# SamsungLabs/fcaf3d

Measured on AMD Instinct MI355X. Metric: scenes/sec fwd+bwd, ScanNet 100k-pt 2cm voxels, 1/2/4/8 MI355X, higher is better.
Workload: dtype f32

## Files before the change

fcaf3d_amd/csrc/conv.hip:

```cpp
#include "fc_common.h"
#include "../../include/fcaf3d_hip.h"
#ifdef FC_TRACE
__device__ unsigned long long* g_trace_buf_lds;
__device__ int g_trace_cap_lds;
extern "C" int fc_debug_trace_lds(unsigned long long* buf, int cap) {
  FC_HIP(hipMemcpyToSymbol(HIP_SYMBOL(g_trace_buf_lds), &buf, sizeof(buf)));
  FC_HIP(hipMemcpyToSymbol(HIP_SYMBOL(g_trace_cap_lds), &cap, sizeof(cap)));
  return FC_OK;
}
#define TR_BUF g_trace_buf_lds
#define TR_CAP g_trace_cap_lds
#endif
#include "fc_trace.h"

typedef float f32x16 __attribute__((ext_vector_type(16)));
typedef float f32x2 __attribute__((ext_vector_type(2)));
typedef float f32x4 __attribute__((ext_vector_type(4)));

__device__ __attribute__((aligned(16))) float g_zero_row[64];

__device__ int g_fc_prio;
extern "C" int fc_debug_set_prio(int mode) {
  FC_HIP(hipMemcpyToSymbol(HIP_SYMBOL(g_fc_prio), &mode, sizeof(mode)));
  return FC_OK;
}

static int g_bf16_fast = 0;
extern "C" int fc_set_bf16_fast(int on) {
  g_bf16_fast = on ? 1 : 0;
  return FC_OK;
}

static int g_split_mode = 2;
static inline int split_mode() { return g_bf16_fast ? 0 : g_split_mode; }
extern "C" int fc_set_split_mode(int mode) {
  if (mode != 0 && mode != 2) return FC_EINVAL;
  g_split_mode = mode;
  return FC_OK;
}
extern "C" int fc_get_split_mode(void) { return split_mode(); }
static int g_h3r = 1;
extern "C" int fc_debug_set_h3r(int mode) {
  if (mode < 0 || mode > 2) return FC_EINVAL;
  g_h3r = mode;
  return FC_OK;
}

#include <mutex>
#include "conv_tile.h"
#include "conv_f32.h"
#include "wgrad_f32.h"
#include "conv_stem.h"
#include "conv_x6.h"
#include "wgrad_x6.h"
#include "conv_h3r.h"
#include "conv_route.h"
static inline RouteEnv route_env() { return {split_mode(), g_bf16_fast, g_h3r}; }

__global__ __launch_bounds__(256) void k_amax(const f32x4* __restrict__ x, int64_t n4, const float* __restrict__ tail, int ntail,
                                              unsigned* __restrict__ slot) {
  __shared__ unsigned wm[4];
  __shared__ int last_s;
  unsigned m = 0u;
  const int64_t stride = (int64_t)gridDim.x * 256;
  for (int64_t i = (int64_t)blockIdx.x * 256 + threadIdx.x; i < n4; i += 4 * stride) {
    f32x4 v[4];
#pragma unroll
    for (int q = 0; q < 4; ++q) v[q] = i + q * stride < n4 ? x[i + q * stride] : f32x4{0.f, 0.f, 0.f, 0.f};
#pragma unroll
    for (int q = 0; q < 4; ++q)
#pragma unroll
      for (int j = 0; j < 4; ++j) { const unsigned u = __float_as_uint(v[q][j]) & 0x7fffffffu; m = (u > m && u < 0x7f800000u) ? u : m; }
  }
  if (blockIdx.x == 0 && (int)threadIdx.x < ntail) { const unsigned u = __float_as_uint(tail[threadIdx.x]) & 0x7fffffffu; m = (u > m && u < 0x7f800000u) ? u : m; }
#pragma unroll
  for (int off = 32; off > 0; off >>= 1) { const unsigned o = (unsigned)__shfl_xor((int)m, off, 64); m = o > m ? o : m; }
  if ((threadIdx.x & 63) == 0) wm[threadIdx.x >> 6] = m;
  __syncthreads();
  if (threadIdx.x == 0) {
    unsigned b = wm[0];
    for (int w = 1; w < 4; ++w) b = wm[w] > b ? wm[w] : b;
    if (b > __hip_atomic_load(&slot[1], __ATOMIC_RELAXED, __HIP_MEMORY_SCOPE_AGENT)) atomicMax(&slot[1], b);
    __threadfence();
    last_s = atomicAdd(&slot[2], 1u) == gridDim.x - 1;
    if (last_s) {
      __threadfence();
      slot[0] = atomicExch(&slot[1], 0u);
      slot[2] = 0u;
    }
  }
}

constexpr int AMAX_RING = 2048;
static unsigned* g_amax_ring[16] = {};
static unsigned g_amax_next[16] = {};
static std::mutex g_amax_ring_mu;
static int amax_ring_slot(unsigned** slot) {
  int dev = 0;
  FC_HIP(hipGetDevice(&dev));
  if (dev < 0 || dev >= 16) return FC_EINVAL;
  std::lock_guard<std::mutex> lock(g_amax_ring_mu);
  if (!g_amax_ring[dev]) {
    FC_HIP(hipMalloc((void**)&g_amax_ring[dev], (size_t)AMAX_RING * FC_AMAX_SLOT_BYTES));
    FC_HIP(hipMemset(g_amax_ring[dev], 0, (size_t)AMAX_RING * FC_AMAX_SLOT_BYTES));
  }
  const unsigned i = __atomic_fetch_add(&g_amax_next[dev], 1u, __ATOMIC_RELAXED) % AMAX_RING;
  *slot = g_amax_ring[dev] + (size_t)i * (FC_AMAX_SLOT_BYTES / 4);
  return FC_OK;
}
static int amax_launch(const float* x, int64_t n, unsigned* slot, hipStream_t stream) {
// ... 410 lines not shown
template <int G>
__global__ __launch_bounds__(256) void k_wgrad_reduce4(const float* __restrict__ part, float* __restrict__ gW, int64_t elems4, int S) {
  __shared__ f32x4 red[256];
  constexpr int COLS = 256 / G;
  const int col = threadIdx.x % COLS, g = threadIdx.x / COLS;
  const int64_t i = (int64_t)blockIdx.x * COLS + col;
  const int per = (S + G - 1) / G;
  const int s0 = g * per, s1 = (s0 + per < S) ? s0 + per : S;
  f32x4 a = {0.f, 0.f, 0.f, 0.f};
  if (i < elems4) {
    const f32x4* src = reinterpret_cast<const f32x4*>(part) + i;
    int sl = s0;
    for (; sl + 4 <= s1; sl += 4) {
      const f32x4 v0 = src[(int64_t)sl * elems4], v1 = src[(int64_t)(sl + 1) * elems4];
      const f32x4 v2 = src[(int64_t)(sl + 2) * elems4], v3 = src[(int64_t)(sl + 3) * elems4];
      a += v0; a += v1; a += v2; a += v3;
    }
    for (; sl < s1; ++sl) a += src[(int64_t)sl * elems4];
  }
  if (G == 1) {
    if (i < elems4) reinterpret_cast<f32x4*>(gW)[i] = a;
    return;
  }
  red[threadIdx.x] = a;
  __syncthreads();
  if (g == 0 && i < elems4) {
    for (int q = 1; q < G; ++q) a += red[q * COLS + col];
    reinterpret_cast<f32x4*>(gW)[i] = a;
  }
}

__global__ void k_transpose_w(const float* __restrict__ W, float* __restrict__ Wt, int K, int Cin, int Cout) {
  __shared__ float tile[32][33];
  int k = blockIdx.z;
  int ci0 = blockIdx.y * 32, co0 = blockIdx.x * 32;
  int tx = threadIdx.x & 31, ty = threadIdx.x >> 5;
  for (int j = ty; j < 32; j += 8) {
    int ci = ci0 + j, co = co0 + tx;
    tile[j][tx] = (ci < Cin && co < Cout) ? W[((int64_t)k * Cin + ci) * Cout + co] : 0.f;
  }
  __syncthreads();
  for (int j = ty; j < 32; j += 8) {
    int co = co0 + j, ci = ci0 + tx;
    if (ci < Cin && co < Cout) Wt[((int64_t)k * Cout + co) * Cin + ci] = tile[tx][j];
  }
}

struct WgradArgs {
  const float *in, *gout; const int *nbr, *row_index, *cnt; float* part;
  int64_t n_out; int K, Cin, Cout; const unsigned *amax_in, *amax_gout; hipStream_t stream;
};
#define FC_LAUNCH(...) __VA_ARGS__<<<grid, 256, 0, a.stream>>>(a.in, a.gout, a.nbr, a.row_index, a.cnt, a.part, a.n_out, a.K, a.Cin, a.Cout, r.rps)
#define FC_LAUNCH_X6T(...) __VA_ARGS__<<<grid, 256, 0, a.stream>>>(a.in, a.gout, a.nbr, a.row_index, a.cnt, a.part, a.n_out, a.K, a.Cin, a.Cout, r.rps, a.amax_in, a.amax_gout, r.wbuf)
#define FC_LAUNCH_TABLE(...) __VA_ARGS__<<<grid, 256, 0, a.stream>>>(a.in, a.gout, a.nbr, a.part, a.n_out, a.K, a.Cin, a.Cout, r.rps)

template <int BM, int BN, int KO, bool PAIRS>
static void launch_wgrad_x6t(const WgradRoute& r, const WgradArgs& a, dim3 grid) {
  if (r.mode == FC_MODE_BF16) FC_LAUNCH_X6T(k_wgrad_x6t<BM, BN, KO, PAIRS, 1>);
  else if (r.mode == FC_MODE_H3) FC_LAUNCH_X6T(k_wgrad_x6t<BM, BN, KO, PAIRS, 2>);
  else FC_LAUNCH_X6T(k_wgrad_x6t<BM, BN, KO, PAIRS>);
}

template <int BM, int BN>
static void launch_wgrad_tile(const WgradRoute& r, const WgradArgs& a, dim3 grid) {
  const bool pairs = r.table == FC_TABLE_PAIRS;
  if (r.family == FC_WFAM_X6T) { if (pairs) launch_wgrad_x6t<BM, BN, 1, true>(r, a, grid); else launch_wgrad_x6t<BM, BN, 1, false>(r, a, grid); }
  else if (r.family == FC_WFAM_MFMA && !pairs && r.bkr == 32) { if (a.nbr) FC_LAUNCH(k_wgrad_mfma<BM, BN, true, 32, false>); else FC_LAUNCH(k_wgrad_mfma<BM, BN, false, 32, false>); }
  else if constexpr (BM == 64) {
    if (r.family == FC_WFAM_MFMA) { if (pairs) FC_LAUNCH(k_wgrad_mfma<64, BN, true, 32, true>); else FC_LAUNCH(k_wgrad_mfma<64, BN, true, 64, false>); }
    else if (pairs) FC_LAUNCH(k_wgrad_mfma_p<BN, true, true>);
    else if (a.nbr) FC_LAUNCH(k_wgrad_mfma_p<BN, true, false>);
    else FC_LAUNCH(k_wgrad_mfma_p<BN, false, false>);
  }
}

static int launch_wgrad(const WgradRoute& r, const WgradArgs& a) {
  const dim3 grid((unsigned)r.S, r.grid_y);
  const bool wide = r.bn == 128;
  if (r.family == FC_WFAM_STEM) {
    const size_t smem = (size_t)(STEM_ROWS * STEM_JP + STEM_ROWS * 64) * sizeof(float);
    k_stem_wgrad<<<(unsigned)r.S, 256, smem, a.stream>>>(a.in, a.gout, a.nbr, a.part, a.n_out, a.K, r.rps);
  } else if (r.family == FC_WFAM_FMA) FC_LAUNCH_TABLE(k_wgrad_fma);
  else if (r.family == FC_WFAM_MULTI) { if (wide) FC_LAUNCH_TABLE(k_wgrad_multi<128, WGRAD_KO>); else FC_LAUNCH_TABLE(k_wgrad_multi<64, WGRAD_KO>); }
  else if (r.ko == WGRAD_KO) { if (wide) launch_wgrad_x6t<64, 128, WGRAD_KO, false>(r, a, grid); else launch_wgrad_x6t<64, 64, WGRAD_KO, false>(r, a, grid); }
  else if (r.bm == 128) { if (wide) launch_wgrad_tile<128, 128>(r, a, grid); else launch_wgrad_tile<128, 64>(r, a, grid); }
  else { if (wide) launch_wgrad_tile<64, 128>(r, a, grid); else launch_wgrad_tile<64, 64>(r, a, grid); }
  FC_CHECK_LAUNCH();
  return FC_OK;
}
#undef FC_LAUNCH
#undef FC_LAUNCH_X6T
#undef FC_LAUNCH_TABLE

extern "C" {

static int wgrad_reduce(const float* part, float* gW, int64_t elems, int S, hipStream_t stream) {
  if (elems % 4 == 0) {
    const int64_t e4 = elems / 4;
    if (S >= 64) k_wgrad_reduce4<16><<<(unsigned)fc_cdiv(e4, 16), 256, 0, stream>>>(part, gW, e4, S);
    else if (S >= 16) k_wgrad_reduce4<4><<<(unsigned)fc_cdiv(e4, 64), 256, 0, stream>>>(part, gW, e4, S);
    else k_wgrad_reduce4<1><<<(unsigned)fc_cdiv(e4, 256), 256, 0, stream>>>(part, gW, e4, S);
  } else {
    k_wgrad_reduce<<<(unsigned)fc_cdiv(elems, 256), 256, 0, stream>>>(part, gW, elems, S);
  }
  FC_CHECK_LAUNCH();
  return FC_OK;
}

int fc_stem_conv_fwd(const float* in, const float* W, const int* nbr, float* out, float* col, int64_t n_in, int64_t n_out,
                     int K, hipStream_t stream) {
  if (n_in < 0 || n_out < 0 || K < 1 || K > 27 || !nbr) return FC_EINVAL;
  if (n_out == 0) return FC_OK;
  size_t smem = (size_t)(STEM_ROWS * STEM_FWD_LDA + 96 * 64) * sizeof(float);
  k_stem_fwd<<<(unsigned)fc_cdiv(n_out, STEM_ROWS), 256, smem, stream>>>(in, W, nbr, out, col, n_out, K);
  FC_CHECK_LAUNCH();
  return FC_OK;
}

static void stem_col_plan(int64_t n_out, int* S, int64_t* rps) {
  int64_t r = fc_cdiv(fc_cdiv(n_out > 0 ? n_out : 1, 192), STEM_ROWS) * STEM_ROWS;
  *rps = r;
  *S = (int)fc_cdiv(n_out > 0 ? n_out : 1, r);
}

int64_t fc_stem_conv_wgrad_ws_bytes(int64_t n_out, int K) {
  int S; int64_t rps;
  stem_col_plan(n_out, &S, &rps);
  return (int64_t)S * K * STEM_CIN * STEM_COUT * (int64_t)sizeof(float);
}

int fc_stem_conv_wgrad(const float* col, const float* gout, float* gW, int64_t n_out, int K, void* ws, int64_t ws_bytes,
                       hipStream_t stream) {
  if (n_out < 0 || K < 1 || K > 27) return FC_EINVAL;
  const int64_t elems = (int64_t)K * STEM_CIN * STEM_COUT;
  if (n_out == 0) {
    FC_HIP(hipMemsetAsync(gW, 0, elems * sizeof(float), stream));
    return FC_OK;
  }
  int S; int64_t rps;
  stem_col_plan(n_out, &S, &rps);
  if (ws_bytes < (int64_t)S * elems * (int64_t)sizeof(float)) return FC_EWS;
  float* part = (S == 1) ? gW : (float*)ws;
  size_t smem = (size_t)(STEM_ROWS * STEM_JP + STEM_ROWS * 64) * sizeof(float);
  k_stem_wgrad_col<<<(unsigned)S, 256, smem, stream>>>(col, gout, part, n_out, K, rps);
  FC_CHECK_LAUNCH();
  if (S > 1) return wgrad_reduce(part, gW, elems, S, stream);
  return FC_OK;
}

int fc_conv_wgrad_route(int64_t n_in, int64_t n_out, int K, int Cin, int Cout, int flags, int table_kind, int* out) {
  if (!out || n_in < 0 || n_out < 0 || K < 1 || Cin < 1 || Cout < 1) return FC_EINVAL;
  const WgradRoute r = wgrad_route({n_in, n_out, K, Cin, Cout}, flags, table_kind, route_env());
  const int f[16] = {r.family, r.bm, r.bn, r.ko, r.bkr, r.table, r.mode, r.S, (int)(r.rps < 0x7fffffff ? r.rps : 0x7fffffff), r.wbuf, (int)r.grid_y};
  for (int i = 0; i < 16; ++i) out[i] = f[i];
  return r.family == FC_WFAM_INVALID ? FC_EINVAL : FC_OK;
}

int64_t fc_conv_wgrad_ws_bytes(int64_t n_out, int K, int Cin, int Cout, int flags) {
  int S = 0;
  for (int table : {FC_TABLE_NONE, FC_TABLE_DENSE, FC_TABLE_PAIRS}) {
    const WgradRoute r = wgrad_route({n_out, n_out, K, Cin, Cout}, flags, table, route_env());
    if (r.family != FC_WFAM_INVALID && r.S > S) S = r.S;
  }
  return (int64_t)S * K * Cin * Cout * (int64_t)sizeof(float);
}

static int conv_wgrad_impl(const float* in, const float* gout, const int* nbr, const int* row_index, const int* cnt,
                           float* gW, int64_t n_in, int64_t n_out, int K, int Cin, int Cout, int flags, void* ws,
                           int64_t ws_bytes, hipStream_t stream) {
  AmaxHintScope hint_scope;
  if (n_in < 0 || n_out < 0 || K < 1 || Cin < 1 || Cout < 1) return FC_EINVAL;
  const int64_t elems = (int64_t)K * Cin * Cout;
  if (n_out == 0) { FC_HIP(hipMemsetAsync(gW, 0, elems * sizeof(float), stream)); return FC_OK; }
  const WgradRoute r = wgrad_route({n_in, n_out, K, Cin, Cout}, flags, cnt ? FC_TABLE_PAIRS : nbr ? FC_TABLE_DENSE : FC_TABLE_NONE, route_env());
  if (r.family == FC_WFAM_INVALID) return FC_EINVAL;
  if (ws_bytes < (int64_t)r.S * elems * (int64_t)sizeof(float)) return FC_EWS;
  WgradArgs a = {in, gout, nbr, row_index, cnt, (r.S == 1) ? gW : (float*)ws, n_out, K, Cin, Cout, nullptr, nullptr, stream};
  int rc = FC_OK;
  if (r.mode == FC_MODE_H3) {
    rc = operand_amax(in, n_in * (int64_t)Cin, 0, stream, &a.amax_in);
    if (rc == FC_OK) rc = operand_amax(gout, n_out * (int64_t)Cout, 1, stream, &a.amax_gout);
  }
  if (rc == FC_OK) rc = launch_wgrad(r, a);
  if (rc == FC_OK && r.S > 1) rc = wgrad_reduce(a.part, gW, elems, r.S, stream);
  return rc;
}

int fc_conv_wgrad(const float* in, const float* gout, const int* nbr, const int* row_index, float* gW, int64_t n_in,
                  int64_t n_out, int K, int Cin, int Cout, int flags, void* ws, int64_t ws_bytes, hipStream_t stream) {
  if (row_index) return FC_EINVAL;
  return conv_wgrad_impl(in, gout, nbr, nullptr, nullptr, gW, n_in, n_out, K, Cin, Cout, flags, ws, ws_bytes, stream);
}

int fc_conv_wgrad_pairs(const float* in, const float* gout, const int* pair_in, const int* pair_out, const int* pair_cnt,
                        float* gW, int64_t n_in, int64_t n_out, int K, int Cin, int Cout, int flags, void* ws,
                        int64_t ws_bytes, hipStream_t stream) {
  if (!pair_in || !pair_out || !pair_cnt) return FC_EINVAL;
  return conv_wgrad_impl(in, gout, pair_in, pair_out, pair_cnt, gW, n_in, n_out, K, Cin, Cout, flags, ws, ws_bytes, stream);
}

int fc_transpose_weight(const float* W, float* Wt, int K, int Cin, int Cout, hipStream_t stream) {
  if (K < 1 || Cin < 1 || Cout < 1 || K > 65535) return FC_EINVAL;
  dim3 grid((unsigned)fc_cdiv(Cout, 32), (unsigned)fc_cdiv(Cin, 32), (unsigned)K);
  k_transpose_w<<<grid, 256, 0, stream>>>(W, Wt, K, Cin, Cout);
  FC_CHECK_LAUNCH();
  return FC_OK;
// ... 4 lines not shown
```

fcaf3d_amd/csrc/conv_route.h:

```cpp
#ifndef FC_CONV_ROUTE_H
#define FC_CONV_ROUTE_H
#include "fc_common.h"
#include "../../include/fcaf3d_hip.h"

struct RouteEnv { int split_mode, bf16_fast, h3r; };
struct ConvShape { int64_t n_in, n_out; int K, Cin, Cout; };

struct ConvRoute {
  int family;
  int bm, bn, wm;
  int S;
  int wsrc, mode, buf, epi;
  unsigned grid[3];
};
struct WgradRoute {
  int family;
  int bm, bn, ko, bkr;
  int table, mode, S;
  int64_t rps;
  int wbuf;
  unsigned grid_y;
};

static inline int flag_bm(int flags) { return (flags >> FC_CONV_BM_SHIFT) & FC_CONV_TILE_MASK; }
static inline int flag_bn(int flags) { return (flags >> FC_CONV_BN_SHIFT) & FC_CONV_TILE_MASK; }
static inline int flag_s(int flags) { return (flags >> FC_CONV_S_SHIFT) & FC_CONV_S_MASK; }
static inline bool below_2gb(uint64_t bytes) { return bytes < (1ull << 31) - 4096u; }

static inline bool stem_shape(int K, int Cin, int Cout, int flags) { return !(flags & FC_CONV_FMA) && Cin == 3 && Cout == 64 && K <= 27; }

static inline int offset_split(int64_t tiles, int K) {
  if (K <= 1 || tiles >= 384) return 1;
  return (int)(1024 / tiles < K ? 1024 / tiles : K);
}

static inline ConvRoute conv_route(const ConvShape& s, int flags, int table, int64_t live_tiles, const RouteEnv& env) {
  const bool stats = (table & FC_TABLE_STATS) != 0;
  table &= ~FC_TABLE_STATS;
  const bool pairs = table == FC_TABLE_PAIRS, gather = table != FC_TABLE_NONE, split = (flags & FC_CONV_SPLIT) != 0;
  const bool image = split && (flags & FC_CONV_IMAGE);
  const bool wt = (flags & FC_CONV_WT) && !image;
  const int64_t n = s.n_out > 0 ? s.n_out : 1;
  const int K = s.K, Cin = s.Cin, Cout = s.Cout;
  ConvRoute r = {};
  r.family = FC_FAM_INVALID;
  r.wsrc = image ? FC_WSRC_IMAGE : wt ? FC_WSRC_FP32_T : FC_WSRC_FP32;
  if (!gather && (K != 1 || s.n_in != s.n_out)) return r;
  if ((flags & FC_CONV_WT) && !gather) return r;
  const bool mfma = Cin % 32 == 0 && Cout % 64 == 0 && (pairs || (!(flags & FC_CONV_FMA) && K <= 32));
  if (pairs && !mfma) return r;
  if (stats && !(mfma && split)) return r;
  r.bn = (Cout % 128 == 0) ? 128 : 64;
  if (pairs) {
    if (flag_bn(flags) == 1) r.bn = 64;
    r.bm = 128;
    r.S = K;
  } else {
    r.bm = (n > 64 && fc_cdiv(n, 128) * (Cout / r.bn) >= 4) ? 128 : 64;
    if (Cout == 64 && fc_cdiv(n, 256) >= 1024 && !split) r.bm = 256;
    const int fbm = flag_bm(flags), fbn = flag_bn(flags);
    if (fbm) r.bm = fbm == 1 ? 64 : (fbm == 2 ? 128 : 256);
    if (fbn && (Cout % (fbn == 1 ? 64 : 128) == 0)) r.bn = fbn == 1 ? 64 : 128;
    if (r.bm == 256) r.bn = 64;
    if (split && mfma && r.bm == 64) r.bm = 128;
    r.S = mfma ? offset_split(fc_cdiv(n, r.bm) * (Cout / r.bn), K) : 1;
    if (flag_s(flags)) r.S = flag_s(flags) > K ? K : flag_s(flags);
  }
  r.wm = r.bm == 256 ? 4 : 2;
  if (stem_shape(K, Cin, Cout, flags) && !(flags & FC_CONV_WT) && table == FC_TABLE_DENSE) { r.family = FC_FAM_STEM; return r; }
  if (!mfma && table != FC_TABLE_SORTED && !(flags & FC_CONV_IMAGE)) r.family = FC_FAM_FMA;
  if (!mfma) return r;
  r.grid[0] = (unsigned)fc_cdiv(n, r.bm), r.grid[1] = (unsigned)(Cout / r.bn), r.grid[2] = (unsigned)r.S;
  if (pairs && live_tiles > 0) r.grid[0] = (unsigned)live_tiles, r.grid[2] = 1;
  if (split) {
// ... 15 lines not shown
  if (r.family == FC_FAM_GLDS && wt) r.family = FC_FAM_MFMA;
  if (r.bm == 64) r.family = FC_FAM_MFMA;
  return r;
}

#define WGRAD_KO 3

static inline WgradRoute wgrad_route(const ConvShape& s, int flags, int table, const RouteEnv& env) {
  const int64_t n = s.n_out > 0 ? s.n_out : 1;
  const int K = s.K, Cin = s.Cin, Cout = s.Cout, fbm = flag_bm(flags), fbn = flag_bn(flags);
  const bool dense = table == FC_TABLE_DENSE, pairs = table == FC_TABLE_PAIRS, split = (flags & FC_CONV_SPLIT) != 0;
  if (pairs) flags &= ~FC_CONV_WGRAD_DEEP;
  WgradRoute r = {};
  r.family = FC_WFAM_INVALID;
  r.table = table, r.ko = 1, r.bkr = 32, r.mode = FC_MODE_FP32;
  if (table == FC_TABLE_SORTED || (table == FC_TABLE_NONE && (K != 1 || s.n_in != s.n_out))) return r;
  const bool mfma = !(flags & FC_CONV_FMA) && Cin % 64 == 0 && Cout % 64 == 0;
  if (pairs && !mfma) return r;
  if (stem_shape(K, Cin, Cout, flags)) {
    r.family = dense ? FC_WFAM_STEM : FC_WFAM_FMA;
    r.rps = 1024, r.S = (int)fc_cdiv(n, 1024), r.grid_y = dense ? 1 : (unsigned)K;
    return r;
  }
  const bool multi = dense && mfma && !(flags & FC_CONV_WGRAD_MULTI_OFF) && K % WGRAD_KO == 0 && n >= 4096 &&
                     (!(flags & FC_CONV_WGRAD_MULTI_FIRST) || (Cin == 64 && n >= 32768));
  const bool x6t = mfma && split && (multi || !dense);
  const int wide = (Cout % 128 == 0) ? 128 : 64;
  r.bm = 64;
  r.bn = wide;
  if (fbm == 2 && Cin % 128 == 0) r.bm = 128;
  if (fbn == 1) r.bn = 64;
  if (fbn == 2 && Cout % 128 == 0) r.bn = 128;
  if (split && !dense && Cin % 128 == 0) r.bm = 128;
  int64_t sp = 1728 / (mfma ? (int64_t)K * (Cin / r.bm) * (Cout / r.bn) : (int64_t)K);
  if (multi) {
    constexpr int round_wide = 256, round_narrow = 512;
    sp = (wide == 128 ? round_wide : round_narrow) / ((int64_t)(K / WGRAD_KO) * (Cin / 64) * (Cout / wide));
  }
  const int64_t max_by_rows = fc_cdiv(n, mfma ? 512 : 2048);
  sp = sp > max_by_rows ? max_by_rows : sp;
  sp = sp > 256 ? 256 : sp < 1 ? 1 : sp;
  if (flag_s(flags)) sp = flag_s(flags);
  r.rps = fc_align(fc_cdiv(n, sp), 64);
  r.S = (int)fc_cdiv(n, r.rps);
  if (!mfma) { r.family = FC_WFAM_FMA, r.grid_y = (unsigned)K; return r; }
  if (x6t) {
    r.family = FC_WFAM_X6T;
    r.mode = env.bf16_fast ? FC_MODE_BF16 : env.split_mode == 2 ? FC_MODE_H3 : FC_MODE_SIX;
    r.bn = wide;
    if (multi) r.bm = 64, r.ko = WGRAD_KO;
    else if (r.bm == 128 && r.bn == 128 && (int64_t)r.S * K * (Cin / 128) * (Cout / 128) < 512) r.bm = 64;
    r.wbuf = !(flags & FC_CONV_FLAT) && below_2gb((uint64_t)s.n_in * (uint64_t)Cin * 4u) && below_2gb((uint64_t)s.n_out * (uint64_t)Cout * 4u) &&
             s.n_in < (1 << 24) && s.n_out < (1 << 24) && below_2gb((uint64_t)K * (uint64_t)s.n_out * 4u);
  } else if (multi) {
    r.family = FC_WFAM_MULTI, r.bm = 64, r.bn = wide, r.ko = WGRAD_KO;
  } else {
    if (pairs) r.bm = 64;
    const bool wpipe = r.bm == 64 && !(flags & FC_CONV_WGRAD_DEEP) && !(flags & FC_CONV_WGRAD_PIPE_OFF) &&
                       ((flags & FC_CONV_WGRAD_PIPE_ON) || (pairs && r.bn == 128));
    r.family = wpipe ? FC_WFAM_MFMA_P : FC_WFAM_MFMA;
    if (!wpipe && dense && (flags & FC_CONV_WGRAD_DEEP) && r.bm == 64) r.bkr = 64;
  }
  r.grid_y = (unsigned)((K / r.ko) * (Cin / r.bm) * (Cout / r.bn));
  return r;
}
#endif
```

fcaf3d_amd/csrc/wgrad_x6.h:

```cpp
#pragma once

#ifdef FC_KO_WG_NOSPLIT
#define WG_SPLIT2(x0, x1, p0, p1, p2) do { p0 = x6_hi2(__float_as_uint(x0), __float_as_uint(x1)); p1 = p0; p2 = p0; } while (0)
#else
#define WG_SPLIT2(x0, x1, p0, p1, p2) x6_split2(x0, x1, p0, p1, p2)
#endif


typedef short x6_s16x4 __attribute__((ext_vector_type(4)));
__device__ __forceinline__ u32x4 x6_tr_frag(const u32x2* base, int unit) {
  const auto p = (__attribute__((address_space(3))) x6_s16x4*)(base + unit);
  const x6_s16x4 lo = __builtin_amdgcn_ds_read_tr16_b64_v4i16(p);
  const x6_s16x4 hi = __builtin_amdgcn_ds_read_tr16_b64_v4i16(p + 32);
  const u32x2 a = __builtin_bit_cast(u32x2, lo), b = __builtin_bit_cast(u32x2, hi);
  u32x4 v = {a[0], a[1], b[0], b[1]};
  return v;
}

template <int BMc, int BNc, int KO, bool PAIRS, int MODE = 0>
__global__ __launch_bounds__(256, (KO * (BMc / 64) * (BNc / 64) >= 6) ? 2 : 3) void k_wgrad_x6t(
    const float* __restrict__ in, const float* __restrict__ gout, const int* __restrict__ nbr,
    const int* __restrict__ row_index, const int* __restrict__ cnt, float* __restrict__ part, int64_t n_out, int K, int Cin,
    int Cout, int64_t rows_per_split, const unsigned* __restrict__ amax_a, const unsigned* __restrict__ amax_g, int buf) {
  constexpr int TM = BMc / 64, TN = BNc / 64;
// ... 177 lines not shown
#pragma unroll
                  for (int j = 0; j < TN; ++j) acc[o][i][j] = H3_MFMA(fa[o][pa][i], fb[pb][j], acc[o][i][j]);
        }
      } else
#pragma unroll
      for (int b = 0; b < 2; ++b) {
        u32x4 fb[3][TN];
#pragma unroll
        for (int pl = 0; pl < 3; ++pl)
#pragma unroll
          for (int j = 0; j < TN; ++j) fb[pl][j] = x6_tr_frag(Gs, (pl * SG + wc * TN + j) * 256 + b * 128 + f_unit);
        u32x4 fa[KO][3][TM];
#pragma unroll
        for (int o = 0; o < KO; ++o)
#pragma unroll
          for (int pl = 0; pl < 3; ++pl)
#pragma unroll
            for (int i = 0; i < TM; ++i) fa[o][pl][i] = x6_tr_frag(As, ((o * 3 + pl) * SA + wr * TM + i) * 256 + b * 128 + f_unit);
#pragma unroll
        for (int pb = 2; pb >= 0; --pb)
#pragma unroll
          for (int pa = 2 - pb; pa >= 0; --pa)
#pragma unroll
            for (int o = 0; o < KO; ++o)
#pragma unroll
              for (int i = 0; i < TM; ++i)
#pragma unroll
                for (int j = 0; j < TN; ++j) {
#ifdef FC_KO_WG_NOMFMA
                  acc[o][i][j][0] += __uint_as_float((fa[o][pa][i][0] ^ fb[pb][j][0]) & 0x3fffffu);
#else
                  acc[o][i][j] = X6_MFMA(fa[o][pa][i], fb[pb][j], acc[o][i][j]);
#endif
                }
      }
    }
  }
#pragma unroll
  for (int o = 0; o < KO; ++o) {
    if (k0 + o >= K) break;
    float* dst = part + ((int64_t)blockIdx.x * K + k0 + o) * Cin * Cout;
#pragma unroll
    for (int i = 0; i < TM; ++i)
#pragma unroll
      for (int j = 0; j < TN; ++j)
#pragma unroll
        for (int e = 0; e < 16; ++e) {
          const int row = ci0 + wr * (BMc / 2) + i * 32 + (e & 3) + 8 * (e >> 2) + 4 * h;
          const int col = co0 + wc * (BNc / 2) + j * 32 + r;
          dst[(int64_t)row * Cout + col] = H3 ? acc[o][i][j][e] * h3_inv : acc[o][i][j][e];
        }
  }
}
```

include/fcaf3d_hip.h:

```cpp
#ifndef FCAF3D_HIP_H
#define FCAF3D_HIP_H
#include <stdint.h>

#ifndef __HIP_PLATFORM_AMD__
typedef struct ihipStream_t* hipStream_t;
#endif

#ifdef __cplusplus
extern "C" {
#endif

#define FC_ABI_VERSION 19
#ifndef FC_AMAX_SLOT_BYTES
#define FC_AMAX_SLOT_BYTES 2048
#endif
int fc_abi_version(void);


int fc_voxelize(const float* points, int64_t n, int pt_stride, int batch_idx, float voxel_size, float feat_div,
                int nfeat, int* coords, float* feats, hipStream_t stream);

int fc_augment_voxelize(const float* points, int64_t n_src, int pt_stride, const int* sample_idx, int64_t n_out,
                        const float* xform_host, int batch_idx, float voxel_size, float feat_div, int nfeat, int* coords,
                        float* feats, float* points_out, hipStream_t stream);
// ... 85 lines not shown
int fc_conv_fwd(const float* in, const float* W, const int* nbr, const int* out_index, float* out, int64_t n_in,
                int64_t n_out, int K, int Cin, int Cout, int flags, void* ws, int64_t ws_bytes, hipStream_t stream);

int64_t fc_conv_fwd_pairs_ws_bytes(int64_t n_out, int K, int Cout);
int fc_conv_fwd_pairs(const float* in, const float* W, const int* pair_in, const int* pair_cnt, const int* pair_pos,
                      float* out, int64_t n_in, int64_t n_out, int K, int Cin, int Cout, int flags, void* ws,
                      int64_t ws_bytes, hipStream_t stream);

int fc_conv_fwd_pairs_tiles(const float* in, const float* W, const int* pair_in, const int* pair_cnt, const int* pair_pos,
                            float* out, int64_t n_in, int64_t n_out, int K, int Cin, int Cout, int64_t live_tiles, int flags,
                            void* ws, int64_t ws_bytes, hipStream_t stream);

int64_t fc_conv_stats_blocks(int64_t n_out, int K, int Cin, int Cout, int flags, int pairs);
int fc_conv_fwd_stats(const float* in, const float* W, const int* nbr, const int* out_index, float* out, int64_t n_in,
                      int64_t n_out, int K, int Cin, int Cout, int flags, void* ws, int64_t ws_bytes, float* stats,
                      hipStream_t stream);
int fc_conv_fwd_pairs_tiles_stats(const float* in, const float* W, const int* pair_in, const int* pair_cnt, const int* pair_pos,
                                  float* out, int64_t n_in, int64_t n_out, int K, int Cin, int Cout, int64_t live_tiles, int flags,
                                  void* ws, int64_t ws_bytes, float* stats, hipStream_t stream);
int fc_conv_fwd_bn_bwd_stats(const float* in, const float* W, const int* nbr, const int* out_index, float* out, int64_t n_in,
                             int64_t n_out, int K, int Cin, int Cout, int flags, void* ws, int64_t ws_bytes, float* stats,
                             const float* bn_x, const float* mean, const float* var, const float* gamma, const float* beta, float eps,
                             int act, const float* add, const float* bn_y, hipStream_t stream);
int fc_conv_fwd_pairs_tiles_bn_bwd_stats(const float* in, const float* W, const int* pair_in, const int* pair_cnt, const int* pair_pos,
                                         float* out, int64_t n_in, int64_t n_out, int K, int Cin, int Cout, int64_t live_tiles, int flags,
                                         void* ws, int64_t ws_bytes, float* stats, const float* bn_x, const float* mean,
                                         const float* var, const float* gamma, const float* beta, float eps, int act,
                                         const float* add, const float* bn_y, hipStream_t stream);

int64_t fc_conv_wgrad_ws_bytes(int64_t n_out, int K, int Cin, int Cout, int flags);
int fc_conv_wgrad(const float* in, const float* gout, const int* nbr, const int* row_index, float* gW, int64_t n_in,
                  int64_t n_out, int K, int Cin, int Cout, int flags, void* ws, int64_t ws_bytes, hipStream_t stream);
int fc_conv_wgrad_pairs(const float* in, const float* gout, const int* pair_in, const int* pair_out, const int* pair_cnt,
                        float* gW, int64_t n_in, int64_t n_out, int K, int Cin, int Cout, int flags, void* ws,
                        int64_t ws_bytes, hipStream_t stream);

int fc_stem_conv_fwd(const float* in, const float* W, const int* nbr, float* out, float* col, int64_t n_in, int64_t n_out,
                     int K, hipStream_t stream);
int64_t fc_stem_conv_wgrad_ws_bytes(int64_t n_out, int K);
int fc_stem_conv_wgrad(const float* col, const float* gout, float* gW, int64_t n_out, int K, void* ws, int64_t ws_bytes,
                       hipStream_t stream);

int fc_transpose_weight(const float* W, float* Wt, int K, int Cin, int Cout, hipStream_t stream);

enum { FC_TABLE_NONE, FC_TABLE_DENSE, FC_TABLE_SORTED, FC_TABLE_PAIRS, FC_TABLE_STATS = 8 };
enum { FC_FAM_INVALID, FC_FAM_STEM, FC_FAM_FMA, FC_FAM_MFMA, FC_FAM_MFMA_P, FC_FAM_GLDS, FC_FAM_X6, FC_FAM_H3R };
enum { FC_WFAM_INVALID, FC_WFAM_STEM, FC_WFAM_FMA, FC_WFAM_MFMA, FC_WFAM_MFMA_P, FC_WFAM_MULTI, FC_WFAM_X6T };
enum { FC_WSRC_FP32, FC_WSRC_FP32_T, FC_WSRC_IMAGE };
enum { FC_MODE_FP32, FC_MODE_SIX, FC_MODE_BF16, FC_MODE_H3 };
enum { FC_EPI_NONE, FC_EPI_KERNEL, FC_EPI_SUM };
enum { FC_ROUTE_FAMILY, FC_ROUTE_BM, FC_ROUTE_BN, FC_ROUTE_WM, FC_ROUTE_S, FC_ROUTE_WSRC, FC_ROUTE_MODE, FC_ROUTE_BUF, FC_ROUTE_EPI,
       FC_ROUTE_GRID_X, FC_ROUTE_GRID_Y, FC_ROUTE_GRID_Z };
enum { FC_WROUTE_FAMILY, FC_WROUTE_BM, FC_WROUTE_BN, FC_WROUTE_KO, FC_WROUTE_BKR, FC_WROUTE_TABLE, FC_WROUTE_MODE, FC_WROUTE_S,
       FC_WROUTE_RPS, FC_WROUTE_WBUF, FC_WROUTE_GRID_Y };
int fc_conv_fwd_route(int64_t n_in, int64_t n_out, int K, int Cin, int Cout, int flags, int table_kind, int64_t live_tiles,
                      int* out);
int fc_conv_wgrad_route(int64_t n_in, int64_t n_out, int K, int Cin, int Cout, int flags, int table_kind, int* out);


int64_t fc_col_stats_ws_bytes(int64_t n, int C, int nseg);
int fc_col_stats(const float* x, const int* seg, int seg_stride, int64_t n, int C, int nseg, float* mean, float* var,
                 float* cnt, void* ws, int64_t ws_bytes, hipStream_t stream);

int fc_seg_col_sums(const float* x, const int* seg, int seg_stride, int64_t n, int C, int nseg, float* out, void* ws,
                    int64_t ws_bytes, hipStream_t stream);
int fc_bn_running_update(const float* mean, const float* var, const float* cnt, float momentum, int C, float* running_mean,
                         float* running_var, long long* num_batches_tracked, hipStream_t stream);

int fc_norm_act_fwd(const float* x, const int* seg, int seg_stride, int64_t n, int C, const float* mean, const float* var,
                    float eps, const float* gamma, const float* beta, const float* residual, int act, float* y,
                    hipStream_t stream);
int64_t fc_norm_act_bwd_ws_bytes(int64_t n, int C, int nseg);
int fc_norm_act_bwd(const float* x, const float* y, const float* gy, const int* seg, int seg_stride, int64_t n, int C,
                    int nseg, const float* mean, const float* var, const float* cnt, float eps, const float* gamma,
                    const float* beta, int act, float* gx, float* gres, float* sums, void* ws, int64_t ws_bytes,
                    hipStream_t stream);

int64_t fc_bn_stats_ws_bytes(int64_t n, int C);
int fc_bn_stats_train(const float* x, int64_t n, int C, float momentum, float* mean, float* var, float* cnt,
                      float* running_mean, float* running_var, long long* num_batches_tracked, void* ws,
                      int64_t ws_bytes, hipStream_t stream);
int64_t fc_bn_small_ws_bytes(int C);
int fc_bn_act_train_fwd(const float* x, int64_t n, int C, float eps, const float* gamma, const float* beta,
                        const float* residual, int act, float momentum, float* y, float* mean, float* var, float* cnt,
                        float* running_mean, float* running_var, long long* num_batches_tracked, void* ws,
                        int64_t ws_bytes, hipStream_t stream);
int fc_bn_act_train_bwd(const float* x, const float* y, const float* gy, int64_t n, int C, const float* mean,
                        const float* var, float eps, const float* gamma, const float* beta, int act, float* gx, float* gres,
                        float* sums, void* ws, int64_t ws_bytes, hipStream_t stream);

int64_t fc_bn_train_ws_bytes(int64_t n, int C);
int fc_bn_train_fwd(const float* x, int64_t n, int C, float eps, const float* gamma, const float* beta, const float* residual,
                    int act, float momentum, float* y, float* mean, float* var, float* cnt, float* running_mean,
                    float* running_var, long long* num_batches_tracked, const float* part, int64_t nb_part, int groups,
                    int64_t small_elems, void* ws, int64_t ws_bytes, hipStream_t stream);
int fc_bn_train_bwd(const float* x, const float* y, const float* gy, const float* gy2, int64_t n, int C, const float* mean,
                    const float* var, const float* cnt, float eps, const float* gamma, const float* beta, int act, float* gx,
                    float* gres, float* sums, const float* part, int64_t nb_part, int64_t small_elems, void* ws, int64_t ws_bytes,
                    hipStream_t stream);

enum { FC_NFORM_TRAIN, FC_NFORM_SMALL, FC_NFORM_SEG };
enum { FC_NSTATS_INVALID, FC_NSTATS_PROLOGUE, FC_NSTATS_PARTIAL_SMALL, FC_NSTATS_PARTIAL, FC_NSTATS_TABLE };
enum { FC_NAPPLY_NONE, FC_NAPPLY_BN1, FC_NAPPLY_BN2, FC_NAPPLY_ROWS };
enum { FC_NAMAX_NONE, FC_NAMAX_FOLDED, FC_NAMAX_PASS };
enum { FC_NRED_INVALID, FC_NRED_TABLE, FC_NRED_PARTIAL, FC_NRED_NONE };
enum { FC_NBAPPLY_NONE, FC_NBAPPLY_PROLOGUE, FC_NBAPPLY_FINAL, FC_NBAPPLY_ROWS };
enum { FC_NROUTE_SUMS, FC_NROUTE_APPLY, FC_NROUTE_AMAX, FC_NROUTE_NP, FC_NROUTE_NB, FC_NROUTE_RPB, FC_NROUTE_CG, FC_NROUTE_THREADS, FC_NROUTE_LDS,
// ... 107 lines not shown
                             int flags, int max_total, int cap, float* out_boxes, float* out_scores, int* out_src,
                             int* out_count, int stride_out, void* ws, int64_t ws_bytes, hipStream_t stream);


#define FC_VOTE_ROTATED 1
#define FC_VOTE_WITH_YAW 2
int fc_vote_boxes(const float* boxes, const float* scores, const int* counts_dev, int nseg, int stride, int max_count,
                  const int* keep, const int* keep_counts_dev, int keep_stride, int max_keep, float vote_thr, int flags,
                  float* out_boxes, int* out_members, hipStream_t stream);


#define FC_EVAL_DET_BOTTOM 1
int64_t fc_eval_match_ws_bytes(int64_t n_det, int64_t n_gt, int n_thr);
int fc_eval_match(const float* det_boxes, int det_dim , const float* det_scores, const int64_t* det_labels,
                  const float* gt_boxes , const int* gt_labels,
                  const int64_t* seg , int n_scenes,
                  int64_t n_det, int64_t n_gt, const double* thr , int n_thr, int flags,
                  float* best_iou, int* best_gt, unsigned char* tp_bits, void* ws, int64_t ws_bytes, hipStream_t stream);


int64_t fc_grad_norm_ws_bytes(int64_t n);
int fc_grad_norm(const float* g, int64_t n, float max_norm, float* out, void* ws, int64_t ws_bytes, hipStream_t stream);
int fc_adamw_step(float* p, const float* g, float* m, float* v, int64_t n, float lr, float beta1, float beta2, float eps,
                  float weight_decay, float bias_correction1, float bias_correction2, const float* norm_and_clip,
                  hipStream_t stream);

#define FC_ADAMW_MAX_RUNS 1024
int64_t fc_adamw_groups_table_bytes(int R);
int fc_adamw_groups_pack(const int64_t* begin, const float* lr_mult, const float* decay_mult, int R, int64_t n, void* out,
                         int64_t out_bytes);
int fc_adamw_step_groups(float* p, const float* g, float* m, float* v, int64_t n, float lr, float beta1, float beta2, float eps,
                         float weight_decay, float bias_correction1, float bias_correction2, const float* norm_and_clip,
                         const void* table_dev, int R, hipStream_t stream);

int fc_adamw_ema_step(float* p, const float* g, float* m, float* v, float* ema, int64_t n, float lr, float beta1, float beta2,
                      float eps, float weight_decay, float bias_correction1, float bias_correction2, const float* norm_and_clip,
                      const void* table_dev, int R, float ema_mu, float ema_keep, hipStream_t stream);
int fc_swap_f32(float* a, float* b, int64_t n, hipStream_t stream);

int fc_grad_accum(float* acc, const float* g, int64_t n, float scale, int first, float* ema, const float* p, float ema_mu,
                  float ema_keep, hipStream_t stream);
int64_t fc_grad_accum_norm_ws_bytes(int64_t n);
int fc_grad_accum_norm(float* g_inout, const float* acc, int64_t n, float scale, float max_norm, float* out2, void* ws,
                       int64_t ws_bytes, hipStream_t stream);

int fc_set_bf16_fast(int on);

int fc_set_split_mode(int mode);
int fc_get_split_mode(void);
int fc_amax(const float* x, int64_t n, unsigned* slot, hipStream_t stream);
int fc_conv_amax_hint(const unsigned* amax_in, const unsigned* amax_gout);
int fc_amax_out_hint(unsigned* amax_word);
int fc_debug_set_h3r(int mode);


int fc_exec_op_words(void);
int64_t fc_exec_probe_read(float* ms, int64_t* meta, int64_t cap);
int fc_exec_map_words(void);
int fc_exec(const int64_t* ops, int64_t op_begin, int64_t op_end, const int64_t* addr, const int64_t* dims, const int64_t* maps,
            const int64_t* streams, const int64_t* ws, const int64_t* ws_bytes, int64_t* ws_need, const int64_t* cfg);

#ifdef __cplusplus
}
#endif
#endif
```

Before: 538.5.

## Add producer/consumer warp-specialized wgrad x6t kernel with 512-thread blocks

Adds a weight-gradient kernel variant where four waves act as producers (gather rows, split to multi-plane format, store to LDS) and four waves act as consumers running the MFMA accumulation on a double-buffered stage. It is routed by default for KO==WGRAD_KO, BN=128 non-bf16 tiles. The aim is to overlap global gathers and splitting with matrix math rather than serializing them in the same waves. The cost is doubled block size, more LDS pressure and a barrier per stage, and producer waves sit idle at the end.

```diff
diff --git a/fcaf3d_amd/csrc/conv.hip b/fcaf3d_amd/csrc/conv.hip
--- a/fcaf3d_amd/csrc/conv.hip
+++ b/fcaf3d_amd/csrc/conv.hip
@@ -43,6 +43,12 @@
 extern "C" int fc_debug_set_h3r(int mode) {
   if (mode < 0 || mode > 2) return FC_EINVAL;
   g_h3r = mode;
+  return FC_OK;
+}
+static int g_wgrad_roles = 1;
+extern "C" int fc_debug_set_wgrad_roles(int mode) {
+  if (mode < 0 || mode > 2) return FC_EINVAL;
+  g_wgrad_roles = mode;
   return FC_OK;
 }
 
@@ -55,7 +61,7 @@
 #include "wgrad_x6.h"
 #include "conv_h3r.h"
 #include "conv_route.h"
-static inline RouteEnv route_env() { return {split_mode(), g_bf16_fast, g_h3r}; }
+static inline RouteEnv route_env() { return {split_mode(), g_bf16_fast, g_h3r, g_wgrad_roles}; }
 
 __global__ __launch_bounds__(256) void k_amax(const f32x4* __restrict__ x, int64_t n4, const float* __restrict__ tail, int ntail,
                                               unsigned* __restrict__ slot) {
@@ -572,11 +578,14 @@
 };
 #define FC_LAUNCH(...) __VA_ARGS__<<<grid, 256, 0, a.stream>>>(a.in, a.gout, a.nbr, a.row_index, a.cnt, a.part, a.n_out, a.K, a.Cin, a.Cout, r.rps)
 #define FC_LAUNCH_X6T(...) __VA_ARGS__<<<grid, 256, 0, a.stream>>>(a.in, a.gout, a.nbr, a.row_index, a.cnt, a.part, a.n_out, a.K, a.Cin, a.Cout, r.rps, a.amax_in, a.amax_gout, r.wbuf)
+#define FC_LAUNCH_X6T_ROLES(...) __VA_ARGS__<<<grid, 512, 0, a.stream>>>(a.in, a.gout, a.nbr, a.row_index, a.cnt, a.part, a.n_out, a.K, a.Cin, a.Cout, r.rps, a.amax_in, a.amax_gout, r.wbuf)
 #define FC_LAUNCH_TABLE(...) __VA_ARGS__<<<grid, 256, 0, a.stream>>>(a.in, a.gout, a.nbr, a.part, a.n_out, a.K, a.Cin, a.Cout, r.rps)
 
 template <int BM, int BN, int KO, bool PAIRS>
 static void launch_wgrad_x6t(const WgradRoute& r, const WgradArgs& a, dim3 grid) {
-  if (r.mode == FC_MODE_BF16) FC_LAUNCH_X6T(k_wgrad_x6t<BM, BN, KO, PAIRS, 1>);
+  if (r.roles && r.mode == FC_MODE_H3) FC_LAUNCH_X6T_ROLES(k_wgrad_x6t_roles<BM, BN, KO, PAIRS, 2>);
+  else if (r.roles && r.mode == FC_MODE_SIX) FC_LAUNCH_X6T_ROLES(k_wgrad_x6t_roles<BM, BN, KO, PAIRS, 0>);
+  else if (r.mode == FC_MODE_BF16) FC_LAUNCH_X6T(k_wgrad_x6t<BM, BN, KO, PAIRS, 1>);
   else if (r.mode == FC_MODE_H3) FC_LAUNCH_X6T(k_wgrad_x6t<BM, BN, KO, PAIRS, 2>);
   else FC_LAUNCH_X6T(k_wgrad_x6t<BM, BN, KO, PAIRS>);
 }
@@ -610,6 +619,7 @@
 }
 #undef FC_LAUNCH
 #undef FC_LAUNCH_X6T
+#undef FC_LAUNCH_X6T_ROLES
 #undef FC_LAUNCH_TABLE
 
 extern "C" {
@@ -671,7 +681,7 @@
 int fc_conv_wgrad_route(int64_t n_in, int64_t n_out, int K, int Cin, int Cout, int flags, int table_kind, int* out) {
   if (!out || n_in < 0 || n_out < 0 || K < 1 || Cin < 1 || Cout < 1) return FC_EINVAL;
   const WgradRoute r = wgrad_route({n_in, n_out, K, Cin, Cout}, flags, table_kind, route_env());
-  const int f[16] = {r.family, r.bm, r.bn, r.ko, r.bkr, r.table, r.mode, r.S, (int)(r.rps < 0x7fffffff ? r.rps : 0x7fffffff), r.wbuf, (int)r.grid_y};
+  const int f[16] = {r.family, r.bm, r.bn, r.ko, r.bkr, r.table, r.mode, r.S, (int)(r.rps < 0x7fffffff ? r.rps : 0x7fffffff), r.wbuf, (int)r.grid_y, r.roles};
   for (int i = 0; i < 16; ++i) out[i] = f[i];
   return r.family == FC_WFAM_INVALID ? FC_EINVAL : FC_OK;
 }
diff --git a/fcaf3d_amd/csrc/conv_route.h b/fcaf3d_amd/csrc/conv_route.h
--- a/fcaf3d_amd/csrc/conv_route.h
+++ b/fcaf3d_amd/csrc/conv_route.h
@@ -3,7 +3,7 @@
 #include "fc_common.h"
 #include "../../include/fcaf3d_hip.h"
 
-struct RouteEnv { int split_mode, bf16_fast, h3r; };
+struct RouteEnv { int split_mode, bf16_fast, h3r, wroles; };
 struct ConvShape { int64_t n_in, n_out; int K, Cin, Cout; };
 
 struct ConvRoute {
@@ -20,6 +20,7 @@
   int64_t rps;
   int wbuf;
   unsigned grid_y;
+  int roles;
 };
 
 static inline int flag_bm(int flags) { return (flags >> FC_CONV_BM_SHIFT) & FC_CONV_TILE_MASK; }
@@ -141,6 +142,7 @@
     else if (r.bm == 128 && r.bn == 128 && (int64_t)r.S * K * (Cin / 128) * (Cout / 128) < 512) r.bm = 64;
     r.wbuf = !(flags & FC_CONV_FLAT) && below_2gb((uint64_t)s.n_in * (uint64_t)Cin * 4u) && below_2gb((uint64_t)s.n_out * (uint64_t)Cout * 4u) &&
              s.n_in < (1 << 24) && s.n_out < (1 << 24) && below_2gb((uint64_t)K * (uint64_t)s.n_out * 4u);
+    r.roles = r.mode != FC_MODE_BF16 && (env.wroles == 2 || (env.wroles == 1 && r.ko == WGRAD_KO && r.bn == 128));
   } else if (multi) {
     r.family = FC_WFAM_MULTI, r.bm = 64, r.bn = wide, r.ko = WGRAD_KO;
   } else {
diff --git a/fcaf3d_amd/csrc/wgrad_x6.h b/fcaf3d_amd/csrc/wgrad_x6.h
--- a/fcaf3d_amd/csrc/wgrad_x6.h
+++ b/fcaf3d_amd/csrc/wgrad_x6.h
@@ -253,3 +253,245 @@
         }
   }
 }
+
+template <int BMc, int BNc, int KO, bool PAIRS, int MODE>
+__global__ __launch_bounds__(512, 2) void k_wgrad_x6t_roles(
+    const float* __restrict__ in, const float* __restrict__ gout, const int* __restrict__ nbr,
+    const int* __restrict__ row_index, const int* __restrict__ cnt, float* __restrict__ part, int64_t n_out, int K, int Cin,
+    int Cout, int64_t rows_per_split, const unsigned* __restrict__ amax_a, const unsigned* __restrict__ amax_g, int buf) {
+  static_assert(MODE != 1, "the bf16-fast mode has no role form");
+  constexpr int TM = BMc / 64, TN = BNc / 64;
+  constexpr int SA = BMc / 32, SG = BNc / 32;
+  constexpr bool H3 = MODE == 2;
+  constexpr int NPL = H3 ? 2 : 3;
+  constexpr int AS_UNITS = KO * NPL * SA * 256, GS_UNITS = NPL * SG * 256, NBUF = 2;
+  __shared__ u32x2 As[NBUF * AS_UNITS];
+  __shared__ u32x2 Gs[NBUF * GS_UNITS];
+  float h3_sa = 1.f, h3_sg = 1.f, h3_inv = 1.f;
+  if (H3) {
+    h3_sa = h3_scale(fc_amax_read(amax_a));
+    h3_sg = h3_scale(fc_amax_read(amax_g));
+    h3_inv = h3_unscale(h3_sa, h3_sg);
+  }
+  const int tid = threadIdx.x, lane = tid & 63;
+  const int wave8 = __builtin_amdgcn_readfirstlane(tid >> 6);
+  const bool producer = wave8 < 4;
+  const int wave = wave8 & 3;
+  const int wr = wave >> 1, wc = wave & 1;
+  const int r = lane & 31, h = lane >> 5;
+  const WgradTile wt = wgrad_tile<BMc, BNc>(Cin, Cout, KO);
+  const int k0 = wt.k0, ci0 = wt.ci0, co0 = wt.co0;
+  const WgradRows rows = wgrad_rows<PAIRS, 32>(cnt, k0, n_out, rows_per_split);
+  const int64_t r_begin = rows.begin, r_end = rows.end;
+
+  f32x16 acc[KO][TM][TN];
+#pragma unroll
+  for (int o = 0; o < KO; ++o)
+#pragma unroll
+    for (int i = 0; i < TM; ++i)
+#pragma unroll
+      for (int j = 0; j < TN; ++j)
+#pragma unroll
+        for (int e = 0; e < 16; ++e) acc[o][i][j][e] = 0.f;
+
+  if (r_begin < r_end) {
+    const int s_row = 8 * wave + (lane >> 3), s_c4 = (lane & 7) * 4;
+    const int s_unit = s_row * 8 + (lane & 7);
+    int ia[KO], ig;
+    const __amdgpu_buffer_rsrc_t rnb = __builtin_amdgcn_make_buffer_rsrc(const_cast<int*>(nbr), 0, 0x7fffffff, 0x00020000);
+    const __amdgpu_buffer_rsrc_t rrx = __builtin_amdgcn_make_buffer_rsrc(const_cast<int*>(row_index), 0, 0x7fffffff, 0x00020000);
+    auto fetch_idx = [&](int64_t rb) {
+      const int64_t row = rb + s_row;
+      const int64_t rc = row < r_end ? row : r_end - 1;
+#pragma unroll
+      for (int o = 0; o < KO; ++o) {
+        const int kk = k0 + o < K ? k0 + o : K - 1;
+        int t;
+        if (buf && nbr) t = (int)__builtin_amdgcn_raw_buffer_load_b32(rnb, (int)((unsigned)rc * 4u), (int)((unsigned)kk * (unsigned)n_out * 4u), 0);
+        else t = nbr ? nbr[(int64_t)kk * n_out + rc] : (int)rc;
+        ia[o] = (row < r_end && k0 + o < K) ? t : -1;
+      }
+      if (PAIRS && buf) ig = row < r_end ? (int)__builtin_amdgcn_raw_buffer_load_b32(rrx, (int)((unsigned)rc * 4u), (int)((unsigned)k0 * (unsigned)n_out * 4u), 0) : -1;
+      else ig = row < r_end ? (PAIRS ? row_index[(int64_t)k0 * n_out + rc] : (int)rc) : -1;
+    };
+    f32x4 av[KO][SA], gv[SG];
+    constexpr unsigned WG_DEAD = 0x80000000u;
+    const __amdgpu_buffer_rsrc_t rg = __builtin_amdgcn_make_buffer_rsrc(const_cast<float*>(gout), 0, (int)WG_DEAD, 0x00020000);
+    const __amdgpu_buffer_rsrc_t ri = __builtin_amdgcn_make_buffer_rsrc(const_cast<float*>(in), 0, (int)WG_DEAD, 0x00020000);
+    const unsigned g_row_bytes = (unsigned)Cout * 4u, a_row_bytes = (unsigned)Cin * 4u;
+    const unsigned g_col_bytes = (unsigned)(co0 + s_c4) * 4u, a_col_bytes = (unsigned)(ci0 + s_c4) * 4u;
+    auto load_rows = [&]() {
+      if (buf) {
+        const unsigned og = ig >= 0 ? __umul24((unsigned)ig, g_row_bytes) + g_col_bytes : WG_DEAD;
+#pragma unroll
+        for (int p = 0; p < SG; ++p) gv[p] = __builtin_bit_cast(f32x4, __builtin_amdgcn_raw_buffer_load_b128(rg, (int)(og + 128u * p), 0, 0));
+#pragma unroll
+        for (int o = 0; o < KO; ++o) {
+          const unsigned oa = ia[o] >= 0 ? __umul24((unsigned)ia[o], a_row_bytes) + a_col_bytes : WG_DEAD;
+#pragma unroll
+          for (int p = 0; p < SA; ++p) av[o][p] = __builtin_bit_cast(f32x4, __builtin_amdgcn_raw_buffer_load_b128(ri, (int)(oa + 128u * p), 0, 0));
+        }
+        return;
+      }
+      const float* gp = ig >= 0 ? gout + (int64_t)ig * Cout + co0 + s_c4 : g_zero_row + s_c4;
+#pragma unroll
+      for (int p = 0; p < SG; ++p) {
+#ifdef FC_KO_WG_NOLOAD
+        gv[p] = f32x4{(float)lane, 1.f, 2.f, (float)p};
+#else
+        gv[p] = *reinterpret_cast<const f32x4*>(gp + (ig >= 0 ? p * 32 : 0));
+#endif
+      }
+#pragma unroll
+      for (int o = 0; o < KO; ++o) {
+        const float* ap = ia[o] >= 0 ? in + (int64_t)ia[o] * Cin + ci0 + s_c4 : g_zero_row + s_c4;
+#pragma unroll
+        for (int p = 0; p < SA; ++p) {
+#ifdef FC_KO_WG_NOLOAD
+          av[o][p] = f32x4{(float)lane, 1.f, (float)o, (float)p};
+#else
+          av[o][p] = *reinterpret_cast<const f32x4*>(ap + (ia[o] >= 0 ? p * 32 : 0));
+#endif
+        }
+      }
+    };
+    if (producer) {
+      fetch_idx(r_begin);
+      load_rows();
+    }
+    const int fi = lane & 15, fg = lane >> 4;
+    const int f_unit = (8 * (fg >> 1) + (fi >> 2)) * 8 + (fg & 1) * 4 + (fi & 3);
+    auto split_store = [&](int ab, int gb) {
+#pragma unroll
+      for (int p = 0; p < SG; ++p) {
+        unsigned q[3][2];
+        if (H3) {
+          h3_split2s(gv[p][0], gv[p][1], h3_sg, q[0][0], q[1][0]);
+          h3_split2s(gv[p][2], gv[p][3], h3_sg, q[0][1], q[1][1]);
+        } else {
+          WG_SPLIT2(gv[p][0], gv[p][1], q[0][0], q[1][0], q[2][0]);
+          WG_SPLIT2(gv[p][2], gv[p][3], q[0][1], q[1][1], q[2][1]);
+        }
+#pragma unroll
+        for (int pl = 0; pl < NPL; ++pl) {
+          u32x2 v = {q[pl][0], q[pl][1]};
+          Gs[gb + (pl * SG + p) * 256 + s_unit] = v;
+        }
+      }
+#pragma unroll
+      for (int o = 0; o < KO; ++o)
+#pragma unroll
+        for (int p = 0; p < SA; ++p) {
+          unsigned q[3][2];
+          if (H3) {
+            h3_split2s(av[o][p][0], av[o][p][1], h3_sa, q[0][0], q[1][0]);
+            h3_split2s(av[o][p][2], av[o][p][3], h3_sa, q[0][1], q[1][1]);
+          } else {
+            WG_SPLIT2(av[o][p][0], av[o][p][1], q[0][0], q[1][0], q[2][0]);
+            WG_SPLIT2(av[o][p][2], av[o][p][3], q[0][1], q[1][1], q[2][1]);
+          }
+#pragma unroll
+          for (int pl = 0; pl < NPL; ++pl) {
+            u32x2 v = {q[pl][0], q[pl][1]};
+            As[ab + ((o * NPL + pl) * SA + p) * 256 + s_unit] = v;
+          }
+        }
+    };
+    auto multiply = [&](int ab, int gb) {
+      if (H3) {
+#pragma unroll
+        for (int b = 0; b < 2; ++b) {
+          u32x4 fb[2][TN];
+#pragma unroll
+          for (int pl = 0; pl < 2; ++pl)
+#pragma unroll
+            for (int j = 0; j < TN; ++j) fb[pl][j] = x6_tr_frag(Gs, gb + (pl * SG + wc * TN + j) * 256 + b * 128 + f_unit);
+          u32x4 fa[KO][2][TM];
+#pragma unroll
+          for (int o = 0; o < KO; ++o)
+#pragma unroll
+            for (int pl = 0; pl < 2; ++pl)
+#pragma unroll
+              for (int i = 0; i < TM; ++i) fa[o][pl][i] = x6_tr_frag(As, ab + ((o * 2 + pl) * SA + wr * TM + i) * 256 + b * 128 + f_unit);
+#pragma unroll
+          for (int pb = 1; pb >= 0; --pb)
+#pragma unroll
+            for (int pa = 1 - pb; pa >= 0; --pa)
+#pragma unroll
+              for (int o = 0; o < KO; ++o)
+#pragma unroll
+                for (int i = 0; i < TM; ++i)
+#pragma unroll
+                  for (int j = 0; j < TN; ++j) acc[o][i][j] = H3_MFMA(fa[o][pa][i], fb[pb][j], acc[o][i][j]);
+        }
+      } else
+#pragma unroll
+      for (int b = 0; b < 2; ++b) {
+        u32x4 fb[3][TN];
+#pragma unroll
+        for (int pl = 0; pl < 3; ++pl)
+#pragma unroll
+          for (int j = 0; j < TN; ++j) fb[pl][j] = x6_tr_frag(Gs, gb + (pl * SG + wc * TN + j) * 256 + b * 128 + f_unit);
+        u32x4 fa[KO][3][TM];
+#pragma unroll
+        for (int o = 0; o < KO; ++o)
+#pragma unroll
+          for (int pl = 0; pl < 3; ++pl)
+#pragma unroll
+            for (int i = 0; i < TM; ++i) fa[o][pl][i] = x6_tr_frag(As, ab + ((o * 3 + pl) * SA + wr * TM + i) * 256 + b * 128 + f_unit);
+#pragma unroll
+        for (int pb = 2; pb >= 0; --pb)
+#pragma unroll
+          for (int pa = 2 - pb; pa >= 0; --pa)
+#pragma unroll
+            for (int o = 0; o < KO; ++o)
+#pragma unroll
+              for (int i = 0; i < TM; ++i)
+#pragma unroll
+                for (int j = 0; j < TN; ++j) {
+#ifdef FC_KO_WG_NOMFMA
+                  acc[o][i][j][0] += __uint_as_float((fa[o][pa][i][0] ^ fb[pb][j][0]) & 0x3fffffu);
+#else
+                  acc[o][i][j] = X6_MFMA(fa[o][pa][i], fb[pb][j], acc[o][i][j]);
+#endif
+                }
+      }
+    };
+    const int n_stage = (int)((r_end - r_begin + 31) / 32);
+    auto stage_rb = [&](int t) { return r_begin + 32 * (int64_t)(t < n_stage ? t : n_stage - 1); };
+    if (producer) {
+      fetch_idx(stage_rb(1));
+      split_store(0, 0);
+      load_rows();
+    }
+    __syncthreads();
+    for (int t = 0; t < n_stage; ++t) {
+      if (producer) {
+        if (t + 1 < n_stage) {
+          fetch_idx(stage_rb(t + 2));
+          split_store(((t + 1) & 1) * AS_UNITS, ((t + 1) & 1) * GS_UNITS);
+          load_rows();
+        }
+      } else {
+        multiply((t & 1) * AS_UNITS, (t & 1) * GS_UNITS);
+      }
+      __syncthreads();
+    }
+  }
+  if (producer) return;
+#pragma unroll
+  for (int o = 0; o < KO; ++o) {
+    if (k0 + o >= K) break;
+    float* dst = part + ((int64_t)blockIdx.x * K + k0 + o) * Cin * Cout;
+#pragma unroll
+    for (int i = 0; i < TM; ++i)
+#pragma unroll
+      for (int j = 0; j < TN; ++j)
+#pragma unroll
+        for (int e = 0; e < 16; ++e) {
+          const int row = ci0 + wr * (BMc / 2) + i * 32 + (e & 3) + 8 * (e >> 2) + 4 * h;
+          const int col = co0 + wc * (BNc / 2) + j * 32 + r;
+          dst[(int64_t)row * Cout + col] = H3 ? acc[o][i][j][e] * h3_inv : acc[o][i][j][e];
+        }
+  }
+}
diff --git a/include/fcaf3d_hip.h b/include/fcaf3d_hip.h
--- a/include/fcaf3d_hip.h
+++ b/include/fcaf3d_hip.h
@@ -161,7 +161,7 @@
 enum { FC_ROUTE_FAMILY, FC_ROUTE_BM, FC_ROUTE_BN, FC_ROUTE_WM, FC_ROUTE_S, FC_ROUTE_WSRC, FC_ROUTE_MODE, FC_ROUTE_BUF, FC_ROUTE_EPI,
        FC_ROUTE_GRID_X, FC_ROUTE_GRID_Y, FC_ROUTE_GRID_Z };
 enum { FC_WROUTE_FAMILY, FC_WROUTE_BM, FC_WROUTE_BN, FC_WROUTE_KO, FC_WROUTE_BKR, FC_WROUTE_TABLE, FC_WROUTE_MODE, FC_WROUTE_S,
-       FC_WROUTE_RPS, FC_WROUTE_WBUF, FC_WROUTE_GRID_Y };
+       FC_WROUTE_RPS, FC_WROUTE_WBUF, FC_WROUTE_GRID_Y, FC_WROUTE_ROLES };
 int fc_conv_fwd_route(int64_t n_in, int64_t n_out, int K, int Cin, int Cout, int flags, int table_kind, int64_t live_tiles,
                       int* out);
 int fc_conv_wgrad_route(int64_t n_in, int64_t n_out, int K, int Cin, int Cout, int flags, int table_kind, int* out);
@@ -375,6 +375,7 @@
 int fc_conv_amax_hint(const unsigned* amax_in, const unsigned* amax_gout);
 int fc_amax_out_hint(unsigned* amax_word);
 int fc_debug_set_h3r(int mode);
+int fc_debug_set_wgrad_roles(int mode);
 
 
 int fc_exec_op_words(void);
```

Measured after the change: 515.5. 4.3% lower.
